# robotseu/ORB_Line_SLAM

Hardware: AMD Instinct MI355X
Metric: stereo frames/s extract+match (ORB+LBD), KITTI 1242x375 (higher is better)
Workload: dtype u8

## Files before the change

### include/orbline.h

```cpp
#ifndef ORBLINE_H
#define ORBLINE_H

#include "orbline_types.h"

#ifdef __cplusplus
extern "C" {
#endif

typedef struct olf_ctx olf_ctx;

const char* olf_last_error(void);
int olf_device_count(void);
int olf_default_params(olf_params* p);

int  olf_ctx_create(const olf_params* p, int width, int height, int max_images, olf_ctx** out);
void olf_ctx_destroy(olf_ctx* ctx);
int  olf_ctx_synchronize(olf_ctx* ctx);
int  olf_ctx_set_input_event(olf_ctx* ctx, void* hip_event);
int  olf_ctx_set_deferred_join(olf_ctx* ctx, int on);
int  olf_stereo_frames_join_dev(olf_ctx* ctx, void* stream);
int  olf_ctx_poll_status(olf_ctx* ctx);

int olf_profile_enable(olf_ctx* ctx, int on);
int olf_profile_reset(olf_ctx* ctx);
// ... 20 lines not shown
                       const olf_keypoint* keys, const float* uright, const float* depth, const uint8_t* desc, const uint64_t* mappoint_ids,
                       int n_lines, const olf_keyline* lines, const float* disparity2, const double* le3, const uint8_t* ldesc,
                       const uint64_t* mapline_ids, uint8_t* out, size_t capacity, size_t* written);
int olf_kf_record_counts(const uint8_t* buf, size_t len, int32_t* n_keys, int32_t* n_lines, size_t* record_bytes);
int olf_kf_record_unpack(const uint8_t* buf, size_t len, uint64_t* frame_id, uint64_t* kf_id, double* timestamp, float* t3, float* quat4,
                         olf_keypoint* keys, float* uright, float* depth, uint8_t* desc, uint64_t* mappoint_ids, olf_keyline* lines,
                         float* disparity2, double* le3, uint8_t* ldesc, uint64_t* mapline_ids);

typedef struct olf_voc olf_voc;
int olf_voc_create(int k, int L, int scoring, int weighting, int n_nodes, const int32_t* parent, const uint8_t* is_leaf, const uint8_t* desc,
                   const double* weight, olf_voc** out);
int olf_voc_load_text(const char* path, olf_voc** out);
void olf_voc_destroy(olf_voc* voc);
int olf_voc_info(const olf_voc* voc, int* k, int* L, int* scoring, int* weighting, int* n_nodes, int* n_words);
int olf_bow_words_dev(olf_ctx* ctx, const olf_voc* voc, const uint8_t* d_desc, int n, int levelsup, int32_t* d_word, double* d_weight,
                      int32_t* d_node, void* stream);
int olf_bow_assemble(const olf_voc* voc, const int32_t* word, const double* weight, const int32_t* node, int n, int32_t* bow_ids,
                     double* bow_vals, int* n_bow, int32_t* fv_nodes, int32_t* fv_offs, int32_t* fv_idx, int* n_fv);
int olf_bow_transform(olf_ctx* ctx, const olf_voc* voc, const uint8_t* desc, int n, int levelsup, int32_t* bow_ids, double* bow_vals,
                      int* n_bow, int32_t* fv_nodes, int32_t* fv_offs, int32_t* fv_idx, int* n_fv);
int olf_search_by_bow_batch_dev(olf_ctx* ctx, const olf_voc* voc, int n_frames, int img_stride, const olf_keypoint* d_kps, const uint8_t* d_desc,
                                const int32_t* d_counts, const uint8_t* d_mp_valid, const uint8_t* d_mp_bad, float nnratio, int check_orientation,
                                int levelsup, int32_t* d_matches, int32_t* d_nmatches, void* stream);

int olf_orb_scale_tables(const olf_ctx* ctx, float* scale, float* inv_scale, float* sigma2, float* inv_sigma2,
                         int32_t* features_per_level);
int olf_orb_level_sizes(const olf_ctx* ctx, int32_t* widths, int32_t* heights);
int olf_orb_capacity(const olf_ctx* ctx);
int olf_orb_extract_strided(olf_ctx* ctx, const uint8_t* image, size_t row_stride, olf_keypoint* kps, uint8_t* desc, int32_t* count);
int olf_orb_extract_dev(olf_ctx* ctx, const uint8_t* d_images, int n_images, olf_keypoint* d_kps, uint8_t* d_desc,
                        int32_t* d_counts, void* stream);
int olf_orb_extract(olf_ctx* ctx, const uint8_t* images, int n_images, olf_keypoint* kps, uint8_t* desc, int32_t* counts);
int olf_orb_pyramid_level(olf_ctx* ctx, int image, int level, int blurred, uint8_t* dst);
int olf_orb_debug_candidates(olf_ctx* ctx, int image, int level, int32_t* xys, int cap, int32_t* count);
int olf_debug_status(olf_ctx* ctx, int32_t* out64);
int olf_debug_status_n(olf_ctx* ctx, int32_t* out, int n);
int olf_debug_lsd_owner(olf_ctx* ctx, int image, uint32_t* out);
int olf_debug_lsd_regions(olf_ctx* ctx, int image, int32_t* start_n, double* angle, int cap, int32_t* count);
int olf_debug_lsd_waves(olf_ctx* ctx, int waves_per_image, int rob_entries);
int olf_debug_lsd_groups(olf_ctx* ctx, int groups);
int olf_debug_lsd_scatter(olf_ctx* ctx, int on);
int olf_debug_lsd_log_cap(olf_ctx* ctx, int entries);
int olf_debug_seed_sort(olf_ctx* ctx, const uint32_t* keys, int n, int kthr, int depth_limit, uint32_t* out, int32_t* out_n);
int olf_debug_seed_sort_mode(olf_ctx* ctx, int mode);
int olf_debug_seed_sort_wide(olf_ctx* ctx, const uint64_t* keys, int n, int64_t kthr, int depth_limit, int full, uint32_t* out, int32_t* out_n);
int olf_debug_lsd_pool(olf_ctx* ctx, int pool_chunks);
int olf_debug_fdiv_sweep(olf_ctx* ctx, uint64_t seed, int blocks, int per_thread, uint64_t* mismatches);
int olf_debug_sqrtq_sweep(olf_ctx* ctx, int count, uint64_t* mismatches);
int olf_debug_align_sweep(olf_ctx* ctx, uint64_t seed, int blocks, int per_thread, uint64_t* out3);

int olf_stereo_points_dev(olf_ctx* ctx, int n_pairs, const olf_keypoint* d_kps, const uint8_t* d_desc, const int32_t* d_counts,
                          float* d_uright, float* d_depth, void* stream);
int olf_stereo_points(olf_ctx* ctx, const uint8_t* images, int n_pairs, olf_keypoint* kps, uint8_t* desc, int32_t* counts,
                      float* uright, float* depth);

int olf_match_bf_dev(olf_ctx* ctx, const uint8_t* d_descA, const int32_t* d_nA, int strideA, int a_step, const uint8_t* d_descB,
                     const int32_t* d_nB, int strideB, int b_step, int n_sets, float nnr, int best_lr, int32_t* d_m12, void* stream);
int olf_match_bf(olf_ctx* ctx, const uint8_t* descA, int nA, const uint8_t* descB, int nB, float nnr, int best_lr, int32_t* m12);
int olf_knn2(olf_ctx* ctx, const uint8_t* descQ, int nQ, const uint8_t* descT, int nT, int32_t* idx0, int32_t* dist0, int32_t* dist1);
int olf_match_candidates_dev(olf_ctx* ctx, const uint8_t* d_descQ, int nQ, const uint8_t* d_descT, int nT, const int32_t* d_cand_offsets,
                             const int32_t* d_cand_idx, uint16_t* d_dist, void* stream);
int olf_match_candidates(olf_ctx* ctx, const uint8_t* descQ, int nQ, const uint8_t* descT, int nT, const int32_t* cand_offsets,
                         const int32_t* cand_idx, uint16_t* dist);
typedef struct olf_frame_view {
    const olf_keypoint* keys;
    const uint8_t* desc;
// ... 95 lines not shown
```

### orb_line_slam_amd/_lib.py

```python
import ctypes as C
import os
import numpy as np

_HERE = os.path.dirname(os.path.abspath(__file__))
LIB_PATH = os.environ.get("OLF_LIB_PATH", os.path.join(_HERE, "csrc", "liborbline_hip.so"))
SYNTH_PATH = os.path.join(_HERE, "csrc", "libolf_synth.so")

OLF_OK, OLF_ERR_INVALID, OLF_ERR_CAPACITY, OLF_ERR_HIP, OLF_ERR_NODEVICE = 0, -1, -2, -3, -4
DESC_BYTES = 32

KEYPOINT_DTYPE = np.dtype([("x", "<f4"), ("y", "<f4"), ("size", "<f4"), ("angle", "<f4"), ("response", "<f4"),
                           ("octave", "<i4"), ("class_id", "<i4")])
KEYLINE_DTYPE = np.dtype([("angle", "<f4"), ("class_id", "<i4"), ("octave", "<i4"), ("pt_x", "<f4"), ("pt_y", "<f4"),
                          ("response", "<f4"), ("size", "<f4"), ("startPointX", "<f4"), ("startPointY", "<f4"),
                          ("endPointX", "<f4"), ("endPointY", "<f4"), ("sPointInOctaveX", "<f4"),
                          ("sPointInOctaveY", "<f4"), ("ePointInOctaveX", "<f4"), ("ePointInOctaveY", "<f4"),
                          ("lineLength", "<f4"), ("numOfPixels", "<i4")])
assert KEYPOINT_DTYPE.itemsize == 28 and KEYLINE_DTYPE.itemsize == 68


class OrbParams(C.Structure):
    _fields_ = [("nfeatures", C.c_int32), ("scale_factor", C.c_float), ("nlevels", C.c_int32),
                ("ini_th_fast", C.c_int32), ("min_th_fast", C.c_int32), ("conv_gauss_sum256", C.c_int32)]

# ... 41 lines not shown

def _torch_runtime_first():
    import importlib.util
    if os.environ.get("OLF_NO_TORCH") or importlib.util.find_spec("torch") is None:
        return
    try:
        import torch
        if torch.cuda.is_available():
            torch.cuda.init()
    except Exception:
        pass


def lib():
    global _lib
    if _lib is None:
        if not os.path.exists(LIB_PATH):
            raise ImportError(f"{LIB_PATH} is missing: build it with `make -C orb_line_slam_amd/csrc` "
                              "(python -c 'import __graft_entry__ as g; g.build()'). There is no CPU fallback.")
        _torch_runtime_first()
        L = C.CDLL(LIB_PATH)
        L.olf_last_error.restype = C.c_char_p
        L.olf_ctx_create.argtypes = [C.POINTER(OlfParams), C.c_int, C.c_int, C.c_int, C.POINTER(C.c_void_p)]
        L.olf_ctx_destroy.argtypes = [C.c_void_p]
        L.olf_ctx_destroy.restype = None
        L.olf_ctx_synchronize.argtypes = [C.c_void_p]
        L.olf_ctx_poll_status.argtypes = [C.c_void_p]
        L.olf_orb_scale_tables.argtypes = [C.c_void_p] + [C.c_void_p] * 5
        L.olf_orb_level_sizes.argtypes = [C.c_void_p, C.c_void_p, C.c_void_p]
        L.olf_orb_capacity.argtypes = [C.c_void_p]
        L.olf_orb_extract_dev.argtypes = [C.c_void_p, C.c_void_p, C.c_int, C.c_void_p, C.c_void_p, C.c_void_p, C.c_void_p]
        L.olf_orb_extract.argtypes = [C.c_void_p, C.c_void_p, C.c_int, C.c_void_p, C.c_void_p, C.c_void_p]
        L.olf_orb_pyramid_level.argtypes = [C.c_void_p, C.c_int, C.c_int, C.c_int, C.c_void_p]
        L.olf_orb_debug_candidates.argtypes = [C.c_void_p, C.c_int, C.c_int, C.c_void_p, C.c_int, C.c_void_p]
        L.olf_stereo_points_dev.argtypes = [C.c_void_p, C.c_int] + [C.c_void_p] * 6
        L.olf_stereo_points.argtypes = [C.c_void_p, C.c_void_p, C.c_int] + [C.c_void_p] * 5
        L.olf_match_bf_dev.argtypes = [C.c_void_p, C.c_void_p, C.c_void_p, C.c_int, C.c_int, C.c_void_p, C.c_void_p, C.c_int, C.c_int,
                                       C.c_int, C.c_float, C.c_int, C.c_void_p, C.c_void_p]
        L.olf_match_bf.argtypes = [C.c_void_p, C.c_void_p, C.c_int, C.c_void_p, C.c_int, C.c_float, C.c_int, C.c_void_p]
        L.olf_knn2.argtypes = [C.c_void_p, C.c_void_p, C.c_int, C.c_void_p, C.c_int, C.c_void_p, C.c_void_p, C.c_void_p]
        L.olf_hamming_matrix.argtypes = [C.c_void_p, C.c_void_p, C.c_int, C.c_void_p, C.c_int, C.c_void_p]
        L.olf_line_capacity.argtypes = [C.c_void_p]
        L.olf_line_extract_dev.argtypes = [C.c_void_p, C.c_void_p, C.c_int] + [C.c_void_p] * 4
        L.olf_line_extract.argtypes = [C.c_void_p, C.c_void_p, C.c_int] + [C.c_void_p] * 3
        L.olf_lbd_compute.argtypes = [C.c_void_p, C.c_void_p, C.c_int] + [C.c_void_p] * 3
        L.olf_lsd_debug_scaled.argtypes = [C.c_void_p, C.c_int] + [C.c_void_p] * 3
        L.olf_stereo_lines_dev.argtypes = [C.c_void_p, C.c_int] + [C.c_void_p] * 7
        L.olf_stereo_lines.argtypes = [C.c_void_p, C.c_int] + [C.c_void_p] * 6
        L.olf_stereo_frames_dev.argtypes = [C.c_void_p, C.c_void_p, C.c_int, C.POINTER(FrameBuffers), C.c_void_p]
        L.olf_stereo_frames.argtypes = [C.c_void_p, C.c_void_p, C.c_int, C.POINTER(FrameBuffers)]
        L.olf_match_candidates.argtypes = [C.c_void_p, C.c_void_p, C.c_int, C.c_void_p, C.c_int, C.c_void_p, C.c_void_p, C.c_void_p]
        L.olf_search_by_projection.argtypes = [C.c_void_p, C.POINTER(FrameViewC), C.POINTER(FrameViewC), C.c_float, C.c_int, C.c_int, C.c_void_p, C.c_void_p]
        L.olf_search_by_projection_match12.argtypes = [C.c_void_p, C.POINTER(FrameViewC), C.POINTER(FrameViewC), C.c_float, C.c_int, C.c_int, C.c_void_p, C.c_void_p, C.c_void_p]
        L.olf_search_by_bow.argtypes = [C.c_void_p, C.POINTER(FrameViewC), C.POINTER(FrameViewC), C.c_float, C.c_int, C.c_void_p, C.c_void_p]
        L.olf_search_for_initialization.argtypes = [C.c_void_p, C.POINTER(FrameViewC), C.POINTER(FrameViewC), C.c_void_p, C.c_int, C.c_float, C.c_int,
                                                    C.c_void_p, C.c_void_p]
        V = C.POINTER(FrameViewC)
        L.olf_is_in_frustum.argtypes = [V, C.c_int, C.c_void_p, C.c_void_p, C.c_void_p, C.c_void_p, C.c_float] + [C.c_void_p] * 4
        L.olf_search_by_projection_kf.argtypes = [C.c_void_p, V, V, C.c_void_p, C.c_float, C.c_int, C.c_int, C.c_void_p, C.c_void_p]
        L.olf_search_by_bow_kf.argtypes = [C.c_void_p, V, V, C.c_float, C.c_int, C.c_void_p, C.c_void_p]
        L.olf_search_for_triangulation.argtypes = [C.c_void_p, V, V, C.c_void_p, C.c_void_p, C.c_int, C.c_int, C.c_void_p, C.c_void_p]
        L.olf_fuse_search.argtypes = [C.c_void_p, V, C.c_int] + [C.c_void_p] * 6 + [C.c_float, C.c_void_p, C.c_void_p, C.c_void_p]
        L.olf_fuse_search_sim3.argtypes = [C.c_void_p, V, C.c_void_p, C.c_int] + [C.c_void_p] * 6 + [C.c_float, C.c_void_p, C.c_void_p]
        L.olf_search_by_projection_sim3.argtypes = [C.c_void_p, V, C.c_void_p, C.c_int] + [C.c_void_p] * 6 + [C.c_float, C.c_void_p, C.c_void_p, C.c_void_p]
        L.olf_search_by_sim3.argtypes = [C.c_void_p, V, V, C.c_void_p, C.c_float, C.c_void_p, C.c_void_p, C.c_float, C.c_void_p, C.c_void_p, C.c_void_p]
        L.olf_search_local_map.argtypes = [C.c_void_p, C.POINTER(FrameViewC), C.c_int, C.c_void_p, C.c_void_p, C.c_void_p, C.c_void_p, C.c_void_p,
# ... 114 lines not shown
```

### orb_line_slam_amd/csrc/api.cpp

```cpp
#include "olf_internal.hpp"
#include "line_internal.hpp"
#include "../../include/orbline.h"
#include <map>
#include <mutex>
#include <cstring>
#include <mutex>

namespace olf {
static thread_local std::string g_err;
void set_error(const std::string& s) { g_err = s; }
}

using namespace olf;

struct olf_ctx {
    olf_params params;
    int W = 0, H = 0, max_images = 0;
    int device = 0;
    hipStream_t stream = nullptr;
    OrbHostTables orb;
    OrbDeviceBufs ob;
    uint8_t* d_images = nullptr;
    olf_keypoint* d_kps = nullptr;
    uint8_t* d_desc = nullptr;
// ... 455 lines not shown
    const size_t npx = (size_t)c->W * c->H, cap = c->orb.geom.outCap;
    OLF_HIP_CHECK(hipMemcpyAsync(c->d_images, images, npx * n_images, hipMemcpyHostToDevice, c->stream));
    OLF_TRY(olf_orb_extract_dev(c, c->d_images, n_images, c->d_kps, c->d_desc, c->d_counts, c->stream));
    OLF_HIP_CHECK(hipMemcpyAsync(kps, c->d_kps, cap * n_images * sizeof(olf_keypoint), hipMemcpyDeviceToHost, c->stream));
    OLF_HIP_CHECK(hipMemcpyAsync(desc, c->d_desc, cap * n_images * OLF_DESC_BYTES, hipMemcpyDeviceToHost, c->stream));
    OLF_HIP_CHECK(hipMemcpyAsync(counts, c->d_counts, n_images * sizeof(int), hipMemcpyDeviceToHost, c->stream));
    OLF_HIP_CHECK(hipStreamSynchronize(c->stream));
    return check_status(c);
}

int olf_orb_extract_strided(olf_ctx* c, const uint8_t* image, size_t row_stride, olf_keypoint* kps, uint8_t* desc, int32_t* count)
{
    if (!c || !image || !kps || !desc || !count || row_stride < (size_t)c->W) { set_error("olf_orb_extract_strided: bad argument"); return OLF_ERR_INVALID; }
    const size_t cap = c->orb.geom.outCap;
    OLF_HIP_CHECK(hipMemcpy2DAsync(c->d_images, c->W, image, row_stride, c->W, c->H, hipMemcpyHostToDevice, c->stream));
    OLF_TRY(olf_orb_extract_dev(c, c->d_images, 1, c->d_kps, c->d_desc, c->d_counts, c->stream));
    OLF_HIP_CHECK(hipMemcpyAsync(count, c->d_counts, sizeof(int), hipMemcpyDeviceToHost, c->stream));
    OLF_HIP_CHECK(hipMemcpyAsync(kps, c->d_kps, cap * sizeof(olf_keypoint), hipMemcpyDeviceToHost, c->stream));
    OLF_HIP_CHECK(hipMemcpyAsync(desc, c->d_desc, cap * OLF_DESC_BYTES, hipMemcpyDeviceToHost, c->stream));
    OLF_HIP_CHECK(hipStreamSynchronize(c->stream));
    return check_status(c);
}

int olf_orb_pyramid_level(olf_ctx* c, int image, int level, int blurred, uint8_t* dst)
{
    if (!c || !dst || image < 0 || image >= c->max_images || level < 0 || level >= c->orb.geom.nlevels) return OLF_ERR_INVALID;
    const LevelGeom& L = c->orb.geom.lv[level];
    const uint8_t* src = (blurred ? c->ob.blur : c->ob.pyr) + (size_t)image * c->orb.geom.pyrBytes + L.offset;
    OLF_HIP_CHECK(hipStreamSynchronize(c->stream));
    OLF_HIP_CHECK(hipMemcpy2D(dst, L.w, src, L.pitch, L.w, L.h, hipMemcpyDeviceToHost));
    return OLF_OK;
}

int olf_debug_status(olf_ctx* c, int32_t* out64)
{
    if (!c || !out64) return OLF_ERR_INVALID;
    OLF_HIP_CHECK(hipDeviceSynchronize());
    OLF_HIP_CHECK(hipMemcpy(out64, c->ob.status, 256, hipMemcpyDeviceToHost));
    return OLF_OK;
}

size_t olf_frames_pack_bound(const olf_ctx* c, int n_pairs)
{
    return c && n_pairs >= 0 ? olf::pack_records_bound(n_pairs, c->orb.geom.outCap, c->line.geom.outCap) : 0;
}

int olf_stereo_points_mask_dev(olf_ctx* c, const float* d_depth, size_t n, uint8_t* d_mask, void* stream)
{
    if (!c || !d_depth || !d_mask) { set_error("olf_stereo_points_mask_dev: null argument"); return OLF_ERR_INVALID; }
    OLF_TRY(check_device(c, "olf_stereo_points_mask_dev"));
    return olf::launch_depth_mask(d_depth, d_mask, n, stream ? (hipStream_t)stream : c->stream);
}

int olf_frames_pack_dev(olf_ctx* c, const olf_frame_buffers* fb, int n_pairs, uint8_t* d_dst, size_t dst_capacity, uint64_t* d_bytes, void* stream)
{
    if (!c || !fb || !d_dst || !d_bytes || n_pairs < 0 || 2 * n_pairs > c->max_images || dst_capacity < 64 + (size_t)16 * n_pairs + 16) {
        set_error("olf_frames_pack_dev: bad argument"); return OLF_ERR_INVALID;
    }
    OLF_TRY(check_device(c, "olf_frames_pack_dev"));
    OLF_TRY(join_if_pending(c, stream ? (hipStream_t)stream : c->stream));
    void* ofs = nullptr;
    OLF_TRY(scratch_get(c, 3, (size_t)8 * n_pairs * sizeof(int) + 64, &ofs));
    return olf::launch_pack_records(*fb, n_pairs, c->orb.geom.outCap, c->line.geom.outCap, d_dst, dst_capacity, static_cast<int*>(ofs),
                                    reinterpret_cast<unsigned long long*>(d_bytes), c->ob.status, stream ? (hipStream_t)stream : c->stream);
}

// ... 656 lines not shown
```

### orb_line_slam_amd/csrc/filters.hip

```cpp
#include "olf_internal.hpp"
#include <algorithm>

namespace olf {

constexpr int SF_TW = 128, SF_TH = 32;
constexpr int SF_INW = (SF_TW + 8) / 4;
constexpr int SF_INH = SF_TH + 6;

__device__ __forceinline__ int sf_reflect(int p, int n)
{
    if (p < 0) p = -p;
    if (p >= n) p = 2 * (n - 1) - p;
    return p;
}

__global__ __launch_bounds__(256) void k_sep7(const uint8_t* __restrict__ src, size_t srcImgStride, int srcPitch, uint8_t* __restrict__ dst,
                                              size_t dstImgStride, int dstPitch, int W, int H, Taps7 taps)
{
    __shared__ uint32_t s_in[SF_INH * SF_INW];
    constexpr int HS = (SF_INH + 1) / 2 + ((((SF_INH + 1) / 2) & 1) ? 0 : 1);
    __shared__ uint32_t s_h[SF_TW * HS];
    const int img = blockIdx.z, x0 = blockIdx.x * SF_TW, y0 = blockIdx.y * SF_TH;
    const uint8_t* s = src + (size_t)img * srcImgStride;
    const bool plain = x0 >= 4 && x0 + SF_TW + 4 <= W && y0 >= 3 && y0 + SF_TH + 3 <= H && ((srcPitch | (int)srcImgStride) & 3) == 0 &&
// ... 47 lines not shown
        return __builtin_amdgcn_udot2(va, vb, c, false);
    };
    uint32_t res[4][4];
#pragma unroll
    for (int c = 0; c < 4; ++c) {
        const uint32_t* hp = s_h + (size_t)(4 * q + c) * HS + (ry0 >> 1);
        const uint32_t D0 = hp[0], D1 = hp[1], D2 = hp[2], D3 = hp[3], D4 = hp[4];
        const uint32_t E0 = __builtin_amdgcn_alignbyte(D1, D0, 2u), E1 = __builtin_amdgcn_alignbyte(D2, D1, 2u);
        const uint32_t E2 = __builtin_amdgcn_alignbyte(D3, D2, 2u), E3 = __builtin_amdgcn_alignbyte(D4, D3, 2u);
        res[0][c] = dot2(D3, t6lo, dot2(D2, t45, dot2(D1, t23, dot2(D0, t01, 32768u))));
        res[1][c] = dot2(D3, t6hi, dot2(E2, t45, dot2(E1, t23, dot2(E0, t01, 32768u))));
        res[2][c] = dot2(D4, t6lo, dot2(D3, t45, dot2(D2, t23, dot2(D1, t01, 32768u))));
        res[3][c] = dot2(D4, t6hi, dot2(E3, t45, dot2(E2, t23, dot2(E1, t01, 32768u))));
    }
    uint8_t* d = dst + (size_t)img * dstImgStride;
#pragma unroll
    for (int rr = 0; rr < 4; ++rr) {
        const int gy = y0 + ry0 + rr;
        if (gy >= H) break;
        const uint32_t a0 = min(res[rr][0] >> 16, 255u), a1 = min(res[rr][1] >> 16, 255u), a2 = min(res[rr][2] >> 16, 255u), a3 = min(res[rr][3] >> 16, 255u);
        uint8_t* o = d + (size_t)gy * dstPitch + gx;
        if (gx + 3 < W && ((reinterpret_cast<uintptr_t>(o) & 3) == 0))
            *reinterpret_cast<uint32_t*>(o) = a0 | (a1 << 8) | (a2 << 16) | (a3 << 24);
        else {
            o[0] = (uint8_t)a0;
            if (gx + 1 < W) o[1] = (uint8_t)a1;
            if (gx + 2 < W) o[2] = (uint8_t)a2;
            if (gx + 3 < W) o[3] = (uint8_t)a3;
        }
    }
}

constexpr int SS_ROWS = 16;
constexpr int SS_BROWS = 8;

__device__ __forceinline__ int ss_reflect(int p, int n) { p = p < 0 ? -p : p; return p >= n ? 2 * (n - 1) - p : p; }

template <bool BORDER, int ROWS>
__device__ __forceinline__ void sep7_strip_body(const int t, const uint8_t* __restrict__ src, size_t srcImgStride, int srcPitch, uint8_t* __restrict__ dst,
                                                size_t dstImgStride, int dstPitch, int W, int H, const Taps7& taps, int nsx, int nsy)
{
    const int nb = BORDER ? 1 + ((W + 3) / 4 - (nsx + 1)) : nsx;
    if (t >= nb * nsy) return;
    const int sy = t / nb, si = t - sy * nb;
    const int sx = BORDER ? (si == 0 ? 0 : nsx + si) : si + 1;
    const int x0 = 4 * sx, y0 = sy * ROWS;
    const uint8_t* s = src + (size_t)blockIdx.y * srcImgStride + (x0 - 4);
    uint8_t* d = dst + (size_t)blockIdx.y * dstImgStride + x0;
    const uint32_t tlo = (uint32_t)taps.t[0] | ((uint32_t)taps.t[1] << 8) | ((uint32_t)taps.t[2] << 16) | ((uint32_t)taps.t[3] << 24);
    const uint32_t thi = (uint32_t)taps.t[4] | ((uint32_t)taps.t[5] << 8) | ((uint32_t)taps.t[6] << 16);
    const uint32_t t01 = (uint32_t)taps.t[0] | ((uint32_t)taps.t[1] << 16), t23 = (uint32_t)taps.t[2] | ((uint32_t)taps.t[3] << 16);
    const uint32_t t45 = (uint32_t)taps.t[4] | ((uint32_t)taps.t[5] << 16), t6lo = (uint32_t)taps.t[6], t6hi = (uint32_t)taps.t[6] << 16;
    typedef unsigned short us2 __attribute__((ext_vector_type(2)));
    auto dot2 = [](uint32_t a, uint32_t b, uint32_t c) -> uint32_t {
        us2 va, vb;
        __builtin_memcpy(&va, &a, 4); __builtin_memcpy(&vb, &b, 4);
        return __builtin_amdgcn_udot2(va, vb, c, false);
    };
    struct Raw { uint32_t w[3]; };
    auto load_row = [&](int y) -> Raw {
        Raw r;
        const uint8_t* row = s + (size_t)ss_reflect(min(y, H + 2), H) * srcPitch;
        if (!BORDER) __builtin_memcpy(r.w, row, 12);
        else {
#pragma unroll
            for (int k = 0; k < 3; ++k) {
                uint32_t v = 0;
#pragma unroll
                for (int b = 0; b < 4; ++b) {
                    const int x = x0 - 4 + 4 * k + b;
                    v |= (uint32_t)row[ss_reflect(min(x, W + 2), W) - (x0 - 4)] << (8 * b);
                }
                r.w[k] = v;
            }
        }
        return r;
    };
    auto hrow = [&](const Raw& r, uint32_t* o) {
        const uint32_t* w = r.w;
        o[0] = __builtin_amdgcn_udot4(__builtin_amdgcn_alignbyte(w[2], w[1], 1u), thi, __builtin_amdgcn_udot4(__builtin_amdgcn_alignbyte(w[1], w[0], 1u), tlo, 0u, false), false);
        o[1] = __builtin_amdgcn_udot4(__builtin_amdgcn_alignbyte(w[2], w[1], 2u), thi, __builtin_amdgcn_udot4(__builtin_amdgcn_alignbyte(w[1], w[0], 2u), tlo, 0u, false), false);
        o[2] = __builtin_amdgcn_udot4(__builtin_amdgcn_alignbyte(w[2], w[1], 3u), thi, __builtin_amdgcn_udot4(__builtin_amdgcn_alignbyte(w[1], w[0], 3u), tlo, 0u, false), false);
        o[3] = __builtin_amdgcn_udot4(w[2], thi, __builtin_amdgcn_udot4(w[1], tlo, 0u, false), false);
    };
    auto pair = [&](const Raw& ra, const Raw& rb, uint32_t* Pj) {
        uint32_t a[4], b[4];
        hrow(ra, a); hrow(rb, b);
#pragma unroll
        for (int c = 0; c < 4; ++c) Pj[c] = a[c] | (b[c] << 16);
    };
    uint32_t P[ROWS / 2 + 3][4];
    Raw nx[4];
    {
        Raw r0 = load_row(y0 - 3), r1 = load_row(y0 - 2), r2 = load_row(y0 - 1), r3 = load_row(y0), r4 = load_row(y0 + 1), r5 = load_row(y0 + 2);
#pragma unroll
        for (int k = 0; k < 4; ++k) nx[k] = load_row(y0 + 3 + k);
        pair(r0, r1, P[0]); pair(r2, r3, P[1]); pair(r4, r5, P[2]);
    }
#pragma unroll
    for (int g = 0; g < ROWS / 4; ++g) {
        const Raw c0 = nx[0], c1 = nx[1], c2 = nx[2], c3 = nx[3];
        if (g + 1 < ROWS / 4) {
#pragma unroll
            for (int k = 0; k < 4; ++k) nx[k] = load_row(y0 + 4 * (g + 1) + 3 + k);
            __builtin_amdgcn_sched_barrier(0);
        }
        pair(c0, c1, P[2 * g + 3]); pair(c2, c3, P[2 * g + 4]);
// ... 281 lines not shown
```

### orb_line_slam_amd/csrc/orb_pyramid.hip

```cpp
#include "olf_internal.hpp"

namespace olf {

__global__ __launch_bounds__(256) void k_ingest(const uint8_t* __restrict__ in, uint8_t* __restrict__ pyr,
                                                int W, int H, int in_pitch, int pitch0, int pyrBytes)
{
    const int img = blockIdx.y;
    const int segs = (W + 15) >> 4;
    const int idx = blockIdx.x * 256 + threadIdx.x;
    if (idx >= segs * H) return;
    const int y = idx / segs, x = (idx - y * segs) * 16;
    const uint8_t* src = in + (size_t)img * H * in_pitch + (size_t)y * in_pitch + x;
    uint4 v = make_uint4(0u, 0u, 0u, 0u);
    if (x + 16 <= W) __builtin_memcpy(&v, src, 16);
    else {
        uint32_t w[4] = {0u, 0u, 0u, 0u};
#pragma unroll
        for (int k = 0; k < 16; ++k)
            if (x + k < W) w[k >> 2] |= (uint32_t)src[k] << (8 * (k & 3));
        v = make_uint4(w[0], w[1], w[2], w[3]);
    }
    *reinterpret_cast<uint4*>(pyr + (size_t)img * pyrBytes + (size_t)y * pitch0 + x) = v;
}

// ... 2 lines not shown
{
    const int img = blockIdx.y;
    const int quads = (L.w + 3) >> 2;
    const int idx = blockIdx.x * 256 + threadIdx.x;
    if (idx >= quads * L.h) return;
    const int dy = idx / quads, dx0 = (idx - dy * quads) * 4;
    const uint8_t* src = pyr + (size_t)img * pyrBytes + P.offset;
    const ResizeCoef cy = ry[L.resizeTabY + dy];
    const int y0 = min(max((int)cy.ofs, 0), P.h - 1), y1 = min(max((int)cy.ofs + 1, 0), P.h - 1);
    const uint8_t* S0 = src + (size_t)y0 * P.pitch;
    const uint8_t* S1 = src + (size_t)y1 * P.pitch;
    const int b0 = cy.a0, b1 = cy.a1;
    uint32_t out = 0;
#pragma unroll
    for (int k = 0; k < 4; ++k) {
        const int dx = dx0 + k;
        if (dx < L.w) {
            const ResizeCoef cx = rx[L.resizeTabX + dx];
            const int sx = cx.ofs, sx1 = min(sx + 1, P.w - 1);
            const int h0 = S0[sx] * cx.a0 + S0[sx1] * cx.a1;
            const int h1 = S1[sx] * cx.a0 + S1[sx1] * cx.a1;
            const int v = (((b0 * (h0 >> 4)) >> 16) + ((b1 * (h1 >> 4)) >> 16) + 2) >> 2;
            out |= (uint32_t)(v & 0xff) << (8 * k);
        }
    }
    *reinterpret_cast<uint32_t*>(pyr + (size_t)img * pyrBytes + L.offset + (size_t)dy * L.pitch + dx0) = out;
}

constexpr int FT_W = 128;
constexpr int FT_EW = 124;
constexpr int FT_INW = (FT_W + 8) / 4;


template <int NT>
__global__ __launch_bounds__(NT) __attribute__((amdgpu_waves_per_eu(8, 8)))
void k_fast_score(const uint8_t* __restrict__ pyr, int pyrBytes, LevelGeom L, int minTh,
                  uint32_t* __restrict__ cells, int* __restrict__ cellCount, int totalCells, int cellCap)
{
    constexpr int FT_H = NT / 8, FT_EH = FT_H - 2, FT_INH = FT_H + 6;
    __shared__ uint32_t tile[FT_INH * FT_INW];
    __shared__ unsigned short s_cand[FT_W * FT_H];
    unsigned short* const s_list = s_cand;
    __shared__ uint8_t s_score[FT_H * FT_W];
    __shared__ int s_nc, s_n;
    const int img = blockIdx.z;
    const int x0 = kMinBorder - 4 + blockIdx.x * FT_EW, y0 = kMinBorder + 2 + blockIdx.y * FT_EH;
    const int xBeg = kMinBorder + 3, yBeg = kMinBorder + 3, xEnd = L.maxBorderX - 3, yEnd = L.maxBorderY - 3;
    const uint8_t* src = pyr + (size_t)img * pyrBytes + L.offset;
    {
        constexpr int NLD = (FT_INH * FT_INW + NT - 1) / NT;
        uint32_t tv[NLD];
#pragma unroll
        for (int k = 0; k < NLD; ++k) {
            const int i = threadIdx.x + k * NT;
            const int r = i / FT_INW, j = i - r * FT_INW;
            const int gy = min(y0 - 3 + r, L.h - 1);
            const int xw = min(x0 - 4 + 4 * j, L.pitch - 4);
            tv[k] = i < FT_INH * FT_INW ? *reinterpret_cast<const uint32_t*>(src + (size_t)gy * L.pitch + xw) : 0u;
        }
#pragma unroll
        for (int k = 0; k < NLD; ++k) { const int i = threadIdx.x + k * NT; if (i < FT_INH * FT_INW) tile[i] = tv[k]; }
    }
    reinterpret_cast<uint4*>(s_score)[threadIdx.x] = make_uint4(0u, 0u, 0u, 0u);
    if (threadIdx.x == 0) { s_nc = 0; s_n = 0; }
    __syncthreads();
    const int q = threadIdx.x & 31, ry0 = (threadIdx.x >> 5) * 4;
    uint32_t w[10][3];
#pragma unroll
    for (int r = 0; r < 10; ++r)
#pragma unroll
        for (int k = 0; k < 3; ++k) w[r][k] = tile[(ry0 + r) * FT_INW + q + k];
    uint32_t hE[10], hO[10];
#pragma unroll
    for (int r = 0; r < 10; ++r) {
        hE[r] = __builtin_amdgcn_perm(w[r][1], w[r][1], 0x0c020c00u);
        hO[r] = __builtin_amdgcn_perm(w[r][1], w[r][1], 0x0c030c01u);
    }
    const uint32_t K = 0x02000200u - (uint32_t)(minTh + 1) * 0x00010001u, C9 = 0x02000200u;
    uint32_t acc = 0;
#pragma unroll
    for (int rr = 0; rr < 4; ++rr) {
        const int c = rr + 3;
        const uint32_t eE = __builtin_amdgcn_perm(w[c][2], w[c][1], 0x0c050c03u), eO = __builtin_amdgcn_perm(w[c][2], w[c][1], 0x0c060c04u);
        const uint32_t wE = __builtin_amdgcn_perm(w[c][1], w[c][0], 0x0c030c01u), wO = __builtin_amdgcn_perm(w[c][1], w[c][0], 0x0c040c02u);
        uint32_t ps[2];
#pragma unroll
        for (int h = 0; h < 2; ++h) {
            const uint32_t V = h ? hO[c] : hE[c], N8 = h ? hO[c - 3] : hE[c - 3], N0 = h ? hO[c + 3] : hE[c + 3], N4 = h ? eO : eE, N12 = h ? wO : wE;
            const uint32_t Bb = K - V, Bd = V + K;
            const uint32_t br = ((N0 + Bb) | (N8 + Bb)) & ((N4 + Bb) | (N12 + Bb));
            const uint32_t dk = ((Bd - N0) | (Bd - N8)) & ((Bd - N4) | (Bd - N12));
            ps[h] = br | dk;
        }
        acc = (acc >> 2) | (ps[0] & C9) | ((ps[1] << 1) & (C9 << 1));
    }
    acc >>= 3;
    {
        uint32_t cols = 0, bm = 0;
#pragma unroll
        for (int p = 0; p < 4; ++p) { const int gx = x0 + 4 * q + p; if (gx >= xBeg && gx < xEnd) cols |= 1u << ((p & 1) + 16 * (p >> 1)); }
#pragma unroll
        for (int rr = 0; rr < 4; ++rr) { const int gy = y0 + ry0 + rr; if (gy >= yBeg && gy < yEnd) bm |= cols << (2 * rr); }
        acc &= bm;
    }
    if (acc) {
        int pos = atomicAdd(&s_nc, __popc(acc));
        while (acc) {
            const int b = __builtin_ctz(acc);
            acc &= acc - 1u;
            const int rr = (b & 15) >> 1, p = (b & 1) + 2 * (b >> 4);
            s_cand[pos++] = (unsigned short)((ry0 + rr) * FT_W + 4 * q + p);
        }
    }
    __syncthreads();
    const uint8_t* tb = reinterpret_cast<const uint8_t*>(tile);
    constexpr int P = FT_INW * 4;
    typedef short s2v __attribute__((ext_vector_type(2)));
    const int nCand = s_nc;
    for (int i0 = 0; i0 < nCand; i0 += NT) {
        const int i = i0 + threadIdx.x;
        int sc = 0, id = 0;
        if (i < nCand) {
            id = s_cand[i];
            const int ty = id / FT_W, tx = id - ty * FT_W;
            const uint8_t* c = tb + (ty + 3) * P + tx + 4;
            const int v = c[0];
            int ring[16];
            ring[0] = c[3 * P];   ring[1] = c[3 * P + 1];   ring[2] = c[2 * P + 2];   ring[3] = c[P + 3];
            ring[4] = c[3];       ring[5] = c[-P + 3];      ring[6] = c[-2 * P + 2];  ring[7] = c[-3 * P + 1];
            ring[8] = c[-3 * P];  ring[9] = c[-3 * P - 1];  ring[10] = c[-2 * P - 2]; ring[11] = c[-P - 3];
            ring[12] = c[-3];     ring[13] = c[P - 3];      ring[14] = c[2 * P - 2];  ring[15] = c[3 * P - 1];
            const s2v vv = {(short)v, (short)v};
            s2v R[8], a[8], b[8];
#pragma unroll
            for (int k = 0; k < 8; ++k) {
                const s2v rr = {(short)ring[k], (short)ring[k + 8]};
                R[k] = vv - rr;
            }
            auto sw = [](s2v x) -> s2v { return __builtin_shufflevector(x, x, 1, 0); };
            s2v bestD = {(short)-1000, (short)-1000};
#pragma unroll
            for (int k = 0; k < 8; ++k) a[k] = __builtin_elementwise_min(R[k], k < 7 ? R[k + 1] : sw(R[0]));
#pragma unroll
            for (int k = 0; k < 8; ++k) b[k] = __builtin_elementwise_min(a[k], k < 6 ? a[k + 2] : sw(a[k - 6]));
#pragma unroll
            for (int k = 0; k < 8; ++k) a[k] = __builtin_elementwise_min(b[k], k < 4 ? b[k + 4] : sw(b[k - 4]));
            const s2v a0s = sw(a[0]);
#pragma unroll
            for (int k = 0; k < 8; ++k) bestD = __builtin_elementwise_max(bestD, __builtin_elementwise_min(R[k], k < 7 ? a[k + 1] : a0s));
            s2v bestB = {(short)1000, (short)1000};
#pragma unroll
            for (int k = 0; k < 8; ++k) a[k] = __builtin_elementwise_max(R[k], k < 7 ? R[k + 1] : sw(R[0]));
#pragma unroll
            for (int k = 0; k < 8; ++k) b[k] = __builtin_elementwise_max(a[k], k < 6 ? a[k + 2] : sw(a[k - 6]));
#pragma unroll
            for (int k = 0; k < 8; ++k) a[k] = __builtin_elementwise_max(b[k], k < 4 ? b[k + 4] : sw(b[k - 4]));
            const s2v a0b = sw(a[0]);
#pragma unroll
            for (int k = 0; k < 8; ++k) bestB = __builtin_elementwise_min(bestB, __builtin_elementwise_max(R[k], k < 7 ? a[k + 1] : a0b));
            const s2v best = __builtin_elementwise_max(bestD, -bestB);
            sc = max((int)best.x, (int)best.y) - 1;
        }
        __syncthreads();
        if (sc >= minTh) {
            s_score[id] = (uint8_t)sc;
            s_list[atomicAdd(&s_n, 1)] = (unsigned short)id;
        }
    }
    __syncthreads();
    const int nC = s_n;
    for (int i = threadIdx.x; i < nC; i += NT) {
        const int id = s_list[i], ty = id / FT_W, tx = id - ty * FT_W;
        if (tx < 2 || tx >= 2 + FT_EW || ty < 1 || ty >= 1 + FT_EH) continue;
        const int cur = s_score[id];
        if (cur == 0) continue;
        const int gx = x0 + tx, gy = y0 + ty;
        const int cj = L.wCellM ? (int)(((uint32_t)(gx - xBeg) * L.wCellM) >> 20) : (gx - xBeg) / L.wCell;
        const int ci = L.hCellM ? (int)(((uint32_t)(gy - yBeg) * L.hCellM) >> 20) : (gy - yBeg) / L.hCell;
        const int lx = (gx - xBeg) - cj * L.wCell, ly = (gy - yBeg) - ci * L.hCell;
        const bool xl = lx > 0, xr = lx < L.wCell - 1 && gx + 1 < xEnd, yu = ly > 0, yd = ly < L.hCell - 1 && gy + 1 < yEnd;
        const uint8_t* sp = s_score + id;
        int nb = 0;
        if (yu) { nb = max(nb, (int)sp[-FT_W]); if (xl) nb = max(nb, (int)sp[-FT_W - 1]); if (xr) nb = max(nb, (int)sp[-FT_W + 1]); }
        if (yd) { nb = max(nb, (int)sp[FT_W]); if (xl) nb = max(nb, (int)sp[FT_W - 1]); if (xr) nb = max(nb, (int)sp[FT_W + 1]); }
        if (xl) nb = max(nb, (int)sp[-1]);
        if (xr) nb = max(nb, (int)sp[1]);
        if (cur > nb) {
            const int cell = L.cellBase + ci * L.nCols + cj;
            const int pos = atomicAdd(&cellCount[(size_t)img * totalCells + cell], 1);
            if (pos < cellCap)
                cells[((size_t)img * totalCells + cell) * cellCap + pos] =
                    ((uint32_t)(gy - kMinBorder) << 20) | ((uint32_t)(gx - kMinBorder) << 8) | (uint32_t)cur;
        }
    }
}

constexpr int CS_MAX = 1024;
__global__ __launch_bounds__(64) void k_cells_sort(const OrbGeom* __restrict__ gp, uint32_t* __restrict__ cells, int* __restrict__ cellCount)
{
    __shared__ uint32_t s_k[CS_MAX];
    const OrbGeom& g = *gp;
    const int img = blockIdx.y, cell = blockIdx.x, lane = threadIdx.x;
    int* cnt = cellCount + (size_t)img * g.totalCells + cell;
    const int n = min(*cnt, g.cellCap);
    if (n == 0) return;
    uint32_t* slot = cells + ((size_t)img * g.totalCells + cell) * g.cellCap;
    if (n <= 64) {
        uint32_t k = lane < n ? slot[lane] : 0xffffffffu;
// ... 97 lines not shown
```

Baseline: 15140.

## Shrink FAST candidate queue, scan score tile for NMS, use perm-based border blur loads

The FAST scoring kernel now uses a fixed 1024-entry candidate queue that is refilled in chunks instead of a full tile-sized list, and drops the second atomic survivor list. Non-max suppression now scans the score tile directly with per-thread 16-byte nonzero bitmasks. This cuts shared memory use and atomic traffic but adds extra barriers when candidates overflow the queue. Separately, the 7-tap blur's border path replaces per-byte reflected loads with three word loads combined through byte-permute selectors, its block-row constant is halved, and a debug blur entry point is added.

New measurement: 15010. No clear change (-0.9%).

```diff
diff --git a/include/orbline.h b/include/orbline.h
--- a/include/orbline.h
+++ b/include/orbline.h
@@ -76,6 +76,7 @@
                         int32_t* d_counts, void* stream);
 int olf_orb_extract(olf_ctx* ctx, const uint8_t* images, int n_images, olf_keypoint* kps, uint8_t* desc, int32_t* counts);
 int olf_orb_pyramid_level(olf_ctx* ctx, int image, int level, int blurred, uint8_t* dst);
+int olf_debug_blur7(olf_ctx* ctx, const uint8_t* src, int w, int h, uint8_t* dst);
 int olf_orb_debug_candidates(olf_ctx* ctx, int image, int level, int32_t* xys, int cap, int32_t* count);
 int olf_debug_status(olf_ctx* ctx, int32_t* out64);
 int olf_debug_status_n(olf_ctx* ctx, int32_t* out, int n);
diff --git a/orb_line_slam_amd/_lib.py b/orb_line_slam_amd/_lib.py
--- a/orb_line_slam_amd/_lib.py
+++ b/orb_line_slam_amd/_lib.py
@@ -97,6 +97,7 @@
         L.olf_orb_extract_dev.argtypes = [C.c_void_p, C.c_void_p, C.c_int, C.c_void_p, C.c_void_p, C.c_void_p, C.c_void_p]
         L.olf_orb_extract.argtypes = [C.c_void_p, C.c_void_p, C.c_int, C.c_void_p, C.c_void_p, C.c_void_p]
         L.olf_orb_pyramid_level.argtypes = [C.c_void_p, C.c_int, C.c_int, C.c_int, C.c_void_p]
+        L.olf_debug_blur7.argtypes = [C.c_void_p, C.c_void_p, C.c_int, C.c_int, C.c_void_p]
         L.olf_orb_debug_candidates.argtypes = [C.c_void_p, C.c_int, C.c_int, C.c_void_p, C.c_int, C.c_void_p]
         L.olf_stereo_points_dev.argtypes = [C.c_void_p, C.c_int] + [C.c_void_p] * 6
         L.olf_stereo_points.argtypes = [C.c_void_p, C.c_void_p, C.c_int] + [C.c_void_p] * 5
diff --git a/orb_line_slam_amd/csrc/api.cpp b/orb_line_slam_amd/csrc/api.cpp
--- a/orb_line_slam_amd/csrc/api.cpp
+++ b/orb_line_slam_amd/csrc/api.cpp
@@ -511,6 +511,21 @@
     return OLF_OK;
 }
 
+int olf_debug_blur7(olf_ctx* c, const uint8_t* src, int w, int h, uint8_t* dst)
+{
+    if (!c || !src || !dst || w < 8 || h < 8 || w > 16384 || h > 16384) { set_error("olf_debug_blur7: bad argument"); return OLF_ERR_INVALID; }
+    OLF_TRY(check_device(c, "olf_debug_blur7"));
+    const size_t pitch = ((size_t)w + 63) & ~(size_t)63, inBytes = ((size_t)w * h + 63) & ~(size_t)63;
+    void* st = nullptr;
+    OLF_TRY(scratch_get(c, 1, inBytes + pitch * h, &st));
+    uint8_t* dS = (uint8_t*)st; uint8_t* dD = dS + inBytes;
+    OLF_HIP_CHECK(hipMemcpyAsync(dS, src, (size_t)w * h, hipMemcpyHostToDevice, c->stream));
+    OLF_TRY(launch_sep7(dS, (size_t)w * h, w, dD, pitch * h, (int)pitch, w, h, c->orb.geom.blurTaps, 1, c->stream));
+    OLF_HIP_CHECK(hipMemcpy2DAsync(dst, w, dD, pitch, w, h, hipMemcpyDeviceToHost, c->stream));
+    OLF_HIP_CHECK(hipStreamSynchronize(c->stream));
+    return OLF_OK;
+}
+
 int olf_debug_status(olf_ctx* c, int32_t* out64)
 {
     if (!c || !out64) return OLF_ERR_INVALID;
diff --git a/orb_line_slam_amd/csrc/filters.hip b/orb_line_slam_amd/csrc/filters.hip
--- a/orb_line_slam_amd/csrc/filters.hip
+++ b/orb_line_slam_amd/csrc/filters.hip
@@ -103,7 +103,7 @@
 }
 
 constexpr int SS_ROWS = 16;
-constexpr int SS_BROWS = 8;
+constexpr int SS_BROWS = 4;
 
 __device__ __forceinline__ int ss_reflect(int p, int n) { p = p < 0 ? -p : p; return p >= n ? 2 * (n - 1) - p : p; }
 
@@ -128,22 +128,29 @@
         __builtin_memcpy(&va, &a, 4); __builtin_memcpy(&vb, &b, 4);
         return __builtin_amdgcn_udot2(va, vb, c, false);
     };
+    int a0 = 0, b0 = 0, c0 = 0;
+    uint32_t selAB[3] = {0u, 0u, 0u}, selC[3] = {0u, 0u, 0u};
+    if (BORDER) {
+        a0 = max(x0 - 4, 0); b0 = min(x0, W - 4); c0 = min(x0 + 4, W - 4);
+#pragma unroll
+        for (int j = 0; j < 12; ++j) {
+            const int r = ss_reflect(min(x0 - 4 + j, W + 2), W);
+            const uint32_t ab = r < a0 + 4 ? (uint32_t)(r - a0) : r < c0 ? (uint32_t)(4 + r - b0) : 0x0cu;
+            const uint32_t cc = (r < a0 + 4 || r < c0) ? 0x0cu : (uint32_t)(r - c0);
+            selAB[j >> 2] |= ab << (8 * (j & 3));
+            selC[j >> 2] |= cc << (8 * (j & 3));
+        }
+    }
     struct Raw { uint32_t w[3]; };
     auto load_row = [&](int y) -> Raw {
         Raw r;
         const uint8_t* row = s + (size_t)ss_reflect(min(y, H + 2), H) * srcPitch;
         if (!BORDER) __builtin_memcpy(r.w, row, 12);
         else {
-#pragma unroll
-            for (int k = 0; k < 3; ++k) {
-                uint32_t v = 0;
-#pragma unroll
-                for (int b = 0; b < 4; ++b) {
-                    const int x = x0 - 4 + 4 * k + b;
-                    v |= (uint32_t)row[ss_reflect(min(x, W + 2), W) - (x0 - 4)] << (8 * b);
-                }
-                r.w[k] = v;
-            }
+            uint32_t A, B, C;
+            __builtin_memcpy(&A, row + (a0 - (x0 - 4)), 4); __builtin_memcpy(&B, row + (b0 - (x0 - 4)), 4); __builtin_memcpy(&C, row + (c0 - (x0 - 4)), 4);
+#pragma unroll
+            for (int k = 0; k < 3; ++k) r.w[k] = __builtin_amdgcn_perm(B, A, selAB[k]) | __builtin_amdgcn_perm(C, C, selC[k]);
         }
         return r;
     };
diff --git a/orb_line_slam_amd/csrc/orb_pyramid.hip b/orb_line_slam_amd/csrc/orb_pyramid.hip
--- a/orb_line_slam_amd/csrc/orb_pyramid.hip
+++ b/orb_line_slam_amd/csrc/orb_pyramid.hip
@@ -58,6 +58,7 @@
 constexpr int FT_INW = (FT_W + 8) / 4;
 
 
+constexpr int FT_QCAP = 1024;
 template <int NT>
 __global__ __launch_bounds__(NT) __attribute__((amdgpu_waves_per_eu(8, 8)))
 void k_fast_score(const uint8_t* __restrict__ pyr, int pyrBytes, LevelGeom L, int minTh,
@@ -65,10 +66,9 @@
 {
     constexpr int FT_H = NT / 8, FT_EH = FT_H - 2, FT_INH = FT_H + 6;
     __shared__ uint32_t tile[FT_INH * FT_INW];
-    __shared__ unsigned short s_cand[FT_W * FT_H];
-    unsigned short* const s_list = s_cand;
+    __shared__ unsigned short s_q[FT_QCAP];
     __shared__ uint8_t s_score[FT_H * FT_W];
-    __shared__ int s_nc, s_n;
+    __shared__ int s_nc;
     const int img = blockIdx.z;
     const int x0 = kMinBorder - 4 + blockIdx.x * FT_EW, y0 = kMinBorder + 2 + blockIdx.y * FT_EH;
     const int xBeg = kMinBorder + 3, yBeg = kMinBorder + 3, xEnd = L.maxBorderX - 3, yEnd = L.maxBorderY - 3;
@@ -88,7 +88,7 @@
         for (int k = 0; k < NLD; ++k) { const int i = threadIdx.x + k * NT; if (i < FT_INH * FT_INW) tile[i] = tv[k]; }
     }
     reinterpret_cast<uint4*>(s_score)[threadIdx.x] = make_uint4(0u, 0u, 0u, 0u);
-    if (threadIdx.x == 0) { s_nc = 0; s_n = 0; }
+    if (threadIdx.x == 0) s_nc = 0;
     __syncthreads();
     const int q = threadIdx.x & 31, ry0 = (threadIdx.x >> 5) * 4;
     uint32_t w[10][3];
@@ -129,77 +129,92 @@
         for (int rr = 0; rr < 4; ++rr) { const int gy = y0 + ry0 + rr; if (gy >= yBeg && gy < yEnd) bm |= cols << (2 * rr); }
         acc &= bm;
     }
-    if (acc) {
-        int pos = atomicAdd(&s_nc, __popc(acc));
-        while (acc) {
+    int pos = 0;
+    auto enqueue = [&](int c0) {
+        while (acc && pos < c0 + FT_QCAP) {
             const int b = __builtin_ctz(acc);
             acc &= acc - 1u;
             const int rr = (b & 15) >> 1, p = (b & 1) + 2 * (b >> 4);
-            s_cand[pos++] = (unsigned short)((ry0 + rr) * FT_W + 4 * q + p);
-        }
+            s_q[pos++ - c0] = (unsigned short)((ry0 + rr) * FT_W + 4 * q + p);
+        }
+    };
+    if (acc) {
+        pos = atomicAdd(&s_nc, __popc(acc));
+        enqueue(0);
     }
     __syncthreads();
     const uint8_t* tb = reinterpret_cast<const uint8_t*>(tile);
     constexpr int P = FT_INW * 4;
     typedef short s2v __attribute__((ext_vector_type(2)));
     const int nCand = s_nc;
-    for (int i0 = 0; i0 < nCand; i0 += NT) {
-        const int i = i0 + threadIdx.x;
-        int sc = 0, id = 0;
-        if (i < nCand) {
-            id = s_cand[i];
-            const int ty = id / FT_W, tx = id - ty * FT_W;
-            const uint8_t* c = tb + (ty + 3) * P + tx + 4;
-            const int v = c[0];
-            int ring[16];
-            ring[0] = c[3 * P];   ring[1] = c[3 * P + 1];   ring[2] = c[2 * P + 2];   ring[3] = c[P + 3];
-            ring[4] = c[3];       ring[5] = c[-P + 3];      ring[6] = c[-2 * P + 2];  ring[7] = c[-3 * P + 1];
-            ring[8] = c[-3 * P];  ring[9] = c[-3 * P - 1];  ring[10] = c[-2 * P - 2]; ring[11] = c[-P - 3];
-            ring[12] = c[-3];     ring[13] = c[P - 3];      ring[14] = c[2 * P - 2];  ring[15] = c[3 * P - 1];
-            const s2v vv = {(short)v, (short)v};
-            s2v R[8], a[8], b[8];
-#pragma unroll
-            for (int k = 0; k < 8; ++k) {
-                const s2v rr = {(short)ring[k], (short)ring[k + 8]};
-                R[k] = vv - rr;
+    for (int c0 = 0;;) {
+        const int nq = min(nCand - c0, FT_QCAP);
+        for (int i0 = 0; i0 < nq; i0 += NT) {
+            const int i = i0 + threadIdx.x;
+            int sc = 0, id = 0;
+            if (i < nq) {
+                id = s_q[i];
+                const int ty = id / FT_W, tx = id - ty * FT_W;
+                const uint8_t* c = tb + (ty + 3) * P + tx + 4;
+                const int v = c[0];
+                int ring[16];
+                ring[0] = c[3 * P];   ring[1] = c[3 * P + 1];   ring[2] = c[2 * P + 2];   ring[3] = c[P + 3];
+                ring[4] = c[3];       ring[5] = c[-P + 3];      ring[6] = c[-2 * P + 2];  ring[7] = c[-3 * P + 1];
+                ring[8] = c[-3 * P];  ring[9] = c[-3 * P - 1];  ring[10] = c[-2 * P - 2]; ring[11] = c[-P - 3];
+                ring[12] = c[-3];     ring[13] = c[P - 3];      ring[14] = c[2 * P - 2];  ring[15] = c[3 * P - 1];
+                const s2v vv = {(short)v, (short)v};
+                s2v R[8], a[8], b[8];
+#pragma unroll
+                for (int k = 0; k < 8; ++k) {
+                    const s2v rr = {(short)ring[k], (short)ring[k + 8]};
+                    R[k] = vv - rr;
+                }
+                auto sw = [](s2v x) -> s2v { return __builtin_shufflevector(x, x, 1, 0); };
+                s2v bestD = {(short)-1000, (short)-1000};
+#pragma unroll
+                for (int k = 0; k < 8; ++k) a[k] = __builtin_elementwise_min(R[k], k < 7 ? R[k + 1] : sw(R[0]));
+#pragma unroll
+                for (int k = 0; k < 8; ++k) b[k] = __builtin_elementwise_min(a[k], k < 6 ? a[k + 2] : sw(a[k - 6]));
+#pragma unroll
+                for (int k = 0; k < 8; ++k) a[k] = __builtin_elementwise_min(b[k], k < 4 ? b[k + 4] : sw(b[k - 4]));
+                const s2v a0s = sw(a[0]);
+#pragma unroll
+                for (int k = 0; k < 8; ++k) bestD = __builtin_elementwise_max(bestD, __builtin_elementwise_min(R[k], k < 7 ? a[k + 1] : a0s));
+                s2v bestB = {(short)1000, (short)1000};
+#pragma unroll
+                for (int k = 0; k < 8; ++k) a[k] = __builtin_elementwise_max(R[k], k < 7 ? R[k + 1] : sw(R[0]));
+#pragma unroll
+                for (int k = 0; k < 8; ++k) b[k] = __builtin_elementwise_max(a[k], k < 6 ? a[k + 2] : sw(a[k - 6]));
+#pragma unroll
+                for (int k = 0; k < 8; ++k) a[k] = __builtin_elementwise_max(b[k], k < 4 ? b[k + 4] : sw(b[k - 4]));
+                const s2v a0b = sw(a[0]);
+#pragma unroll
+                for (int k = 0; k < 8; ++k) bestB = __builtin_elementwise_min(bestB, __builtin_elementwise_max(R[k], k < 7 ? a[k + 1] : a0b));
+                const s2v best = __builtin_elementwise_max(bestD, -bestB);
+                sc = max((int)best.x, (int)best.y) - 1;
             }
-            auto sw = [](s2v x) -> s2v { return __builtin_shufflevector(x, x, 1, 0); };
-            s2v bestD = {(short)-1000, (short)-1000};
-#pragma unroll
-            for (int k = 0; k < 8; ++k) a[k] = __builtin_elementwise_min(R[k], k < 7 ? R[k + 1] : sw(R[0]));
-#pragma unroll
-            for (int k = 0; k < 8; ++k) b[k] = __builtin_elementwise_min(a[k], k < 6 ? a[k + 2] : sw(a[k - 6]));
-#pragma unroll
-            for (int k = 0; k < 8; ++k) a[k] = __builtin_elementwise_min(b[k], k < 4 ? b[k + 4] : sw(b[k - 4]));
-            const s2v a0s = sw(a[0]);
-#pragma unroll
-            for (int k = 0; k < 8; ++k) bestD = __builtin_elementwise_max(bestD, __builtin_elementwise_min(R[k], k < 7 ? a[k + 1] : a0s));
-            s2v bestB = {(short)1000, (short)1000};
-#pragma unroll
-            for (int k = 0; k < 8; ++k) a[k] = __builtin_elementwise_max(R[k], k < 7 ? R[k + 1] : sw(R[0]));
-#pragma unroll
-            for (int k = 0; k < 8; ++k) b[k] = __builtin_elementwise_max(a[k], k < 6 ? a[k + 2] : sw(a[k - 6]));
-#pragma unroll
-            for (int k = 0; k < 8; ++k) a[k] = __builtin_elementwise_max(b[k], k < 4 ? b[k + 4] : sw(b[k - 4]));
-            const s2v a0b = sw(a[0]);
-#pragma unroll
-            for (int k = 0; k < 8; ++k) bestB = __builtin_elementwise_min(bestB, __builtin_elementwise_max(R[k], k < 7 ? a[k + 1] : a0b));
-            const s2v best = __builtin_elementwise_max(bestD, -bestB);
-            sc = max((int)best.x, (int)best.y) - 1;
-        }
+            if (sc >= minTh) s_score[id] = (uint8_t)sc;
+        }
+        c0 += FT_QCAP;
+        if (c0 >= nCand) break;
         __syncthreads();
-        if (sc >= minTh) {
-            s_score[id] = (uint8_t)sc;
-            s_list[atomicAdd(&s_n, 1)] = (unsigned short)id;
-        }
+        enqueue(c0);
+        __syncthreads();
     }
     __syncthreads();
-    const int nC = s_n;
-    for (int i = threadIdx.x; i < nC; i += NT) {
-        const int id = s_list[i], ty = id / FT_W, tx = id - ty * FT_W;
-        if (tx < 2 || tx >= 2 + FT_EW || ty < 1 || ty >= 1 + FT_EH) continue;
+    const int ty = threadIdx.x >> 3, tx0 = (threadIdx.x & 7) * 16;
+    uint32_t cm = 0;
+    if (ty >= 1 && ty < 1 + FT_EH) {
+        const uint4 sv = reinterpret_cast<const uint4*>(s_score)[threadIdx.x];
+        auto nz4 = [](uint32_t w) -> uint32_t { return ((((((w & 0x7f7f7f7fu) + 0x7f7f7f7fu) | w) & 0x80808080u) >> 7) * 0x00204081u >> 21) & 0xfu; };
+        cm = nz4(sv.x) | (nz4(sv.y) << 4) | (nz4(sv.z) << 8) | (nz4(sv.w) << 12);
+        if (tx0 == 0) cm &= ~3u;
+        if (tx0 + 16 == FT_W) cm &= 0x3fffu;
+    }
+    while (cm) {
+        const int tx = tx0 + __builtin_ctz(cm), id = ty * FT_W + tx;
+        cm &= cm - 1u;
         const int cur = s_score[id];
-        if (cur == 0) continue;
         const int gx = x0 + tx, gy = y0 + ty;
         const int cj = L.wCellM ? (int)(((uint32_t)(gx - xBeg) * L.wCellM) >> 20) : (gx - xBeg) / L.wCell;
         const int ci = L.hCellM ? (int)(((uint32_t)(gy - yBeg) * L.hCellM) >> 20) : (gy - yBeg) / L.hCell;
```
